# apple/ml-stable-diffusion

Hardware: NVIDIA H100
Metric: diffusion_iter_per_s (higher is better)
Workload: dtype f16

## Files before the change

### ml-stable-diffusion_b200/csrc/common.cuh

```cuda
#pragma once

#include <cuda.h>
#include <cuda_bf16.h>
#include <cuda_fp16.h>
#include <cuda_runtime.h>
#include <stdint.h>
#include <stdio.h>
#include <string.h>

namespace b200sd {

void set_error(const char* fmt, ...);

#define B200SD_CHECK_CUDA(expr)                                                            \
    do {                                                                                   \
        cudaError_t _e = (expr);                                                           \
        if (_e != cudaSuccess) {                                                           \
            ::b200sd::set_error("%s failed: %s (%s:%d)", #expr, cudaGetErrorString(_e),    \
                                __FILE__, __LINE__);                                       \
            return 1;                                                                      \
        }                                                                                  \
    } while (0)

#define B200SD_REQUIRE(cond, ...)                                                          \
    do {                                                                                   \
        if (!(cond)) {                                                                     \
            ::b200sd::set_error(__VA_ARGS__);                                              \
            return 2;                                                                      \
        }                                                                                  \
    } while (0)

int encode_tmap_f16(CUtensorMap* map, const void* base, int rank, const uint64_t* dims,
                    const uint64_t* strides_bytes, const uint32_t* box, const uint32_t* elem_strides);
int encode_tmap(CUtensorMap* map, CUtensorMapDataType dtype, const void* base, int rank, const uint64_t* dims,
                const uint64_t* strides_bytes, const uint32_t* box, const uint32_t* elem_strides,
                CUtensorMapSwizzle swizzle = CU_TENSOR_MAP_SWIZZLE_128B);

int num_sms();

bool pdl_enabled();

bool launch_class_enabled(int cls);

#ifdef __CUDACC__
template <typename... KArgs, typename... Args>
inline cudaError_t launch_kernel(void (*kernel)(KArgs...), dim3 grid, dim3 block, size_t smem, cudaStream_t stream,
                                 Args&&... args) {
    cudaLaunchConfig_t cfg;
    memset(&cfg, 0, sizeof(cfg));
    cfg.gridDim = grid;
    cfg.blockDim = block;
    cfg.dynamicSmemBytes = smem;
    cfg.stream = stream;
    cudaLaunchAttribute attr[1];
    if (pdl_enabled()) {
        attr[0].id = cudaLaunchAttributeProgrammaticStreamSerialization;
        attr[0].val.programmaticStreamSerializationAllowed = 1;
        cfg.attrs = attr;
        cfg.numAttrs = 1;
    }
    return cudaLaunchKernelEx(&cfg, kernel, static_cast<KArgs>(args)...);
}

__device__ __forceinline__ void pdl_wait() { asm volatile("griddepcontrol.wait;" ::: "memory"); }
__device__ __forceinline__ void pdl_trigger() { asm volatile("griddepcontrol.launch_dependents;" ::: "memory"); }

__device__ __forceinline__ uint32_t smem_u32(const void* p) {
    return static_cast<uint32_t>(__cvta_generic_to_shared(p));
}

__device__ __forceinline__ bool elect_one() {
    uint32_t pred = 0;
    asm volatile(
        "{\n\t"
        ".reg .pred P;\n\t"
        "elect.sync _|P, 0xffffffff;\n\t"
        "selp.u32 %0, 1, 0, P;\n\t"
        "}\n"
        : "=r"(pred));
    return pred != 0;
}

__device__ __forceinline__ void mbar_init(uint64_t* bar, uint32_t count) {
    asm volatile("mbarrier.init.shared::cta.b64 [%0], %1;" ::"r"(smem_u32(bar)), "r"(count));
}
__device__ __forceinline__ void fence_barrier_init() {
    asm volatile("fence.mbarrier_init.release.cluster;" ::: "memory");
}
__device__ __forceinline__ void fence_proxy_async_smem() {
    asm volatile("fence.proxy.async.shared::cta;" ::: "memory");
}
__device__ __forceinline__ void mbar_expect_tx(uint64_t* bar, uint32_t bytes) {
    asm volatile("mbarrier.arrive.expect_tx.shared::cta.b64 _, [%0], %1;" ::"r"(smem_u32(bar)), "r"(bytes)
                 : "memory");
}
__device__ __forceinline__ void mbar_arrive(uint64_t* bar) {
    asm volatile("mbarrier.arrive.shared::cta.b64 _, [%0];" ::"r"(smem_u32(bar)) : "memory");
}
__device__ __forceinline__ bool mbar_try_wait(uint64_t* bar, uint32_t parity) {
    uint32_t ok;
    asm volatile(
        "{\n\t"
        ".reg .pred P;\n\t"
        "mbarrier.try_wait.parity.shared::cta.b64 P, [%1], %2;\n\t"
        "selp.u32 %0, 1, 0, P;\n\t"
        "}\n"
        : "=r"(ok)
        : "r"(smem_u32(bar)), "r"(parity)
        : "memory");
    return ok != 0;
}
__device__ __forceinline__ void mbar_wait(uint64_t* bar, uint32_t parity) {
    while (!mbar_try_wait(bar, parity)) {
    }
}

__device__ __forceinline__ void prefetch_tmap(const CUtensorMap* m) {
    asm volatile("prefetch.tensormap [%0];" ::"l"(reinterpret_cast<uint64_t>(m)) : "memory");
}

static constexpr uint64_t kEvictNormal = 0x1000000000000000ull;
static constexpr uint64_t kEvictFirst = 0x12F0000000000000ull;
static constexpr uint64_t kEvictLast = 0x14F0000000000000ull;

__device__ __forceinline__ void tma_load_2d(void* smem_dst, const CUtensorMap* map, uint64_t* bar, int c0, int c1,
                                            uint64_t hint) {
    asm volatile(
        "cp.async.bulk.tensor.2d.shared::cluster.global.mbarrier::complete_tx::bytes.L2::cache_hint"
        " [%0], [%1, {%3, %4}], [%2], %5;" ::"r"(smem_u32(smem_dst)),
        "l"(reinterpret_cast<uint64_t>(map)), "r"(smem_u32(bar)), "r"(c0), "r"(c1), "l"(hint)
        : "memory");
}
__device__ __forceinline__ void tma_load_3d(void* smem_dst, const CUtensorMap* map, uint64_t* bar, int c0, int c1,
                                            int c2, uint64_t hint) {
    asm volatile(
        "cp.async.bulk.tensor.3d.shared::cluster.global.mbarrier::complete_tx::bytes.L2::cache_hint"
        " [%0], [%1, {%3, %4, %5}], [%2], %6;" ::"r"(smem_u32(smem_dst)),
        "l"(reinterpret_cast<uint64_t>(map)), "r"(smem_u32(bar)), "r"(c0), "r"(c1), "r"(c2), "l"(hint)
        : "memory");
}
__device__ __forceinline__ void tma_load_4d(void* smem_dst, const CUtensorMap* map, uint64_t* bar, int c0, int c1,
                                            int c2, int c3, uint64_t hint) {
    asm volatile(
        "cp.async.bulk.tensor.4d.shared::cluster.global.mbarrier::complete_tx::bytes.L2::cache_hint"
        " [%0], [%1, {%3, %4, %5, %6}], [%2], %7;" ::"r"(smem_u32(smem_dst)),
        "l"(reinterpret_cast<uint64_t>(map)), "r"(smem_u32(bar)), "r"(c0), "r"(c1), "r"(c2), "r"(c3), "l"(hint)
        : "memory");
}

__device__ __forceinline__ void wgmma_fence() { asm volatile("wgmma.fence.sync.aligned;" ::: "memory"); }
__device__ __forceinline__ void wgmma_commit() { asm volatile("wgmma.commit_group.sync.aligned;" ::: "memory"); }
template <int N>
__device__ __forceinline__ void wgmma_wait() {
    asm volatile("wgmma.wait_group.sync.aligned %0;" ::"n"(N) : "memory");
}
template <int N>
__device__ __forceinline__ void setmaxnreg_dec() {
    asm volatile("setmaxnreg.dec.sync.aligned.u32 %0;" ::"n"(N));
}
template <int N>
__device__ __forceinline__ void setmaxnreg_inc() {
    asm volatile("setmaxnreg.inc.sync.aligned.u32 %0;" ::"n"(N));
}
template <int R>
__device__ __forceinline__ void wgmma_fence_regs(float* d) {
#pragma unroll
    for (int i = 0; i < R; ++i) asm volatile("" : "+f"(d[i])::"memory");
}

#define B200SD_F8(i) "+f"(d[i]), "+f"(d[i + 1]), "+f"(d[i + 2]), "+f"(d[i + 3]), "+f"(d[i + 4]), "+f"(d[i + 5]), "+f"(d[i + 6]), "+f"(d[i + 7])
template <int N, typename T = __half>
__device__ __forceinline__ void wgmma_ss(float* d, uint64_t da, uint64_t db, uint32_t acc);
#define B200SD_WGMMA_SS(N, T, TY, REGS, IP, IA, IB, ...)                                                             \
    template <>                                                                                                      \
    __device__ __forceinline__ void wgmma_ss<N, T>(float* d, uint64_t da, uint64_t db, uint32_t acc) {               \
        asm volatile("{\n\t.reg .pred p;\n\tsetp.ne.b32 p, %" #IP ", 0;\n\t"                                          \
                     "wgmma.mma_async.sync.aligned.m64n" #N "k16.f32." TY "." TY " {" REGS "}, %" #IA ", %" #IB        \
                     ", p, 1, 1, 0, 0;\n\t}\n"                                                                         \
                     : __VA_ARGS__                                                                                   \
                     : "l"(da), "l"(db), "r"(acc)                                                                    \
                     : "memory");                                                                                    \
    }
#define B200SD_WGMMA_SS_BOTH(N, REGS, IP, IA, IB, ...)                  \
    B200SD_WGMMA_SS(N, __half, "f16", REGS, IP, IA, IB, __VA_ARGS__)   \
    B200SD_WGMMA_SS(N, __nv_bfloat16, "bf16", REGS, IP, IA, IB, __VA_ARGS__)
B200SD_WGMMA_SS_BOTH(16,
                     "%0, %1, %2, %3, %4, %5, %6, %7",
                     10, 8, 9, B200SD_F8(0))
B200SD_WGMMA_SS_BOTH(32,
                     "%0, %1, %2, %3, %4, %5, %6, %7, %8, %9, %10, %11, %12, %13, %14, %15",
                     18, 16, 17, B200SD_F8(0), B200SD_F8(8))
B200SD_WGMMA_SS_BOTH(64,
                     "%0, %1, %2, %3, %4, %5, %6, %7, %8, %9, %10, %11, %12, %13, %14, %15, "
                     "%16, %17, %18, %19, %20, %21, %22, %23, %24, %25, %26, %27, %28, %29, %30, %31",
                     34, 32, 33, B200SD_F8(0), B200SD_F8(8), B200SD_F8(16), B200SD_F8(24))
B200SD_WGMMA_SS_BOTH(96,
                     "%0, %1, %2, %3, %4, %5, %6, %7, %8, %9, %10, %11, %12, %13, %14, %15, "
                     "%16, %17, %18, %19, %20, %21, %22, %23, %24, %25, %26, %27, %28, %29, %30, %31, "
                     "%32, %33, %34, %35, %36, %37, %38, %39, %40, %41, %42, %43, %44, %45, %46, %47",
                     50, 48, 49, B200SD_F8(0), B200SD_F8(8), B200SD_F8(16), B200SD_F8(24), B200SD_F8(32), B200SD_F8(40))
B200SD_WGMMA_SS_BOTH(128,
                     "%0, %1, %2, %3, %4, %5, %6, %7, %8, %9, %10, %11, %12, %13, %14, %15, "
                     "%16, %17, %18, %19, %20, %21, %22, %23, %24, %25, %26, %27, %28, %29, %30, %31, "
                     "%32, %33, %34, %35, %36, %37, %38, %39, %40, %41, %42, %43, %44, %45, %46, %47, "
                     "%48, %49, %50, %51, %52, %53, %54, %55, %56, %57, %58, %59, %60, %61, %62, %63",
                     66, 64, 65, B200SD_F8(0), B200SD_F8(8), B200SD_F8(16), B200SD_F8(24), B200SD_F8(32), B200SD_F8(40), B200SD_F8(48), B200SD_F8(56))
B200SD_WGMMA_SS_BOTH(160,
                     "%0, %1, %2, %3, %4, %5, %6, %7, %8, %9, %10, %11, %12, %13, %14, %15, "
                     "%16, %17, %18, %19, %20, %21, %22, %23, %24, %25, %26, %27, %28, %29, %30, %31, "
                     "%32, %33, %34, %35, %36, %37, %38, %39, %40, %41, %42, %43, %44, %45, %46, %47, "
                     "%48, %49, %50, %51, %52, %53, %54, %55, %56, %57, %58, %59, %60, %61, %62, %63, "
                     "%64, %65, %66, %67, %68, %69, %70, %71, %72, %73, %74, %75, %76, %77, %78, %79",
                     82, 80, 81, B200SD_F8(0), B200SD_F8(8), B200SD_F8(16), B200SD_F8(24), B200SD_F8(32), B200SD_F8(40), B200SD_F8(48), B200SD_F8(56), B200SD_F8(64), B200SD_F8(72))
B200SD_WGMMA_SS_BOTH(192,
                     "%0, %1, %2, %3, %4, %5, %6, %7, %8, %9, %10, %11, %12, %13, %14, %15, "
                     "%16, %17, %18, %19, %20, %21, %22, %23, %24, %25, %26, %27, %28, %29, %30, %31, "
                     "%32, %33, %34, %35, %36, %37, %38, %39, %40, %41, %42, %43, %44, %45, %46, %47, "
                     "%48, %49, %50, %51, %52, %53, %54, %55, %56, %57, %58, %59, %60, %61, %62, %63, "
                     "%64, %65, %66, %67, %68, %69, %70, %71, %72, %73, %74, %75, %76, %77, %78, %79, "
                     "%80, %81, %82, %83, %84, %85, %86, %87, %88, %89, %90, %91, %92, %93, %94, %95",
                     98, 96, 97, B200SD_F8(0), B200SD_F8(8), B200SD_F8(16), B200SD_F8(24), B200SD_F8(32), B200SD_F8(40), B200SD_F8(48), B200SD_F8(56), B200SD_F8(64), B200SD_F8(72), B200SD_F8(80), B200SD_F8(88))
B200SD_WGMMA_SS_BOTH(256,
                     "%0, %1, %2, %3, %4, %5, %6, %7, %8, %9, %10, %11, %12, %13, %14, %15, "
                     "%16, %17, %18, %19, %20, %21, %22, %23, %24, %25, %26, %27, %28, %29, %30, %31, "
                     "%32, %33, %34, %35, %36, %37, %38, %39, %40, %41, %42, %43, %44, %45, %46, %47, "
                     "%48, %49, %50, %51, %52, %53, %54, %55, %56, %57, %58, %59, %60, %61, %62, %63, "
                     "%64, %65, %66, %67, %68, %69, %70, %71, %72, %73, %74, %75, %76, %77, %78, %79, "
                     "%80, %81, %82, %83, %84, %85, %86, %87, %88, %89, %90, %91, %92, %93, %94, %95, "
                     "%96, %97, %98, %99, %100, %101, %102, %103, %104, %105, %106, %107, %108, %109, %110, %111, "
                     "%112, %113, %114, %115, %116, %117, %118, %119, %120, %121, %122, %123, %124, %125, %126, %127",
                     130, 128, 129, B200SD_F8(0), B200SD_F8(8), B200SD_F8(16), B200SD_F8(24), B200SD_F8(32), B200SD_F8(40), B200SD_F8(48), B200SD_F8(56), B200SD_F8(64), B200SD_F8(72), B200SD_F8(80), B200SD_F8(88), B200SD_F8(96), B200SD_F8(104), B200SD_F8(112), B200SD_F8(120))
#undef B200SD_WGMMA_SS_BOTH
#undef B200SD_WGMMA_SS

template <int N>
__device__ __forceinline__ void wgmma_ss_s8(int32_t* d, uint64_t da, uint64_t db, uint32_t acc);
#define B200SD_I8(i) "+r"(d[i]), "+r"(d[i + 1]), "+r"(d[i + 2]), "+r"(d[i + 3]), "+r"(d[i + 4]), "+r"(d[i + 5]), "+r"(d[i + 6]), "+r"(d[i + 7])
#define B200SD_WGMMA_S8(N, REGS, IP, IA, IB, ...)                                                                    \
    template <>                                                                                                      \
    __device__ __forceinline__ void wgmma_ss_s8<N>(int32_t* d, uint64_t da, uint64_t db, uint32_t acc) {             \
        asm volatile("{\n\t.reg .pred p;\n\tsetp.ne.b32 p, %" #IP ", 0;\n\t"                                          \
                     "wgmma.mma_async.sync.aligned.m64n" #N "k32.s32.s8.s8 {" REGS "}, %" #IA ", %" #IB ", p;\n\t}\n"  \
                     : __VA_ARGS__                                                                                   \
                     : "l"(da), "l"(db), "r"(acc)                                                                    \
                     : "memory");                                                                                    \
    }
#define B200SD_R16 "%0, %1, %2, %3, %4, %5, %6, %7"
#define B200SD_R32 B200SD_R16 ", %8, %9, %10, %11, %12, %13, %14, %15"
#define B200SD_R64 B200SD_R32 ", %16, %17, %18, %19, %20, %21, %22, %23, %24, %25, %26, %27, %28, %29, %30, %31"
#define B200SD_R96 B200SD_R64 ", %32, %33, %34, %35, %36, %37, %38, %39, %40, %41, %42, %43, %44, %45, %46, %47"
#define B200SD_R128 B200SD_R96 ", %48, %49, %50, %51, %52, %53, %54, %55, %56, %57, %58, %59, %60, %61, %62, %63"
#define B200SD_R160 B200SD_R128 ", %64, %65, %66, %67, %68, %69, %70, %71, %72, %73, %74, %75, %76, %77, %78, %79"
#define B200SD_R192 B200SD_R160 ", %80, %81, %82, %83, %84, %85, %86, %87, %88, %89, %90, %91, %92, %93, %94, %95"
#define B200SD_R256 B200SD_R192 ", %96, %97, %98, %99, %100, %101, %102, %103, %104, %105, %106, %107, %108, %109, %110, " \
    "%111, %112, %113, %114, %115, %116, %117, %118, %119, %120, %121, %122, %123, %124, %125, %126, %127"
B200SD_WGMMA_S8(16, B200SD_R16, 10, 8, 9, B200SD_I8(0))
B200SD_WGMMA_S8(32, B200SD_R32, 18, 16, 17, B200SD_I8(0), B200SD_I8(8))
B200SD_WGMMA_S8(64, B200SD_R64, 34, 32, 33, B200SD_I8(0), B200SD_I8(8), B200SD_I8(16), B200SD_I8(24))
B200SD_WGMMA_S8(96, B200SD_R96, 50, 48, 49, B200SD_I8(0), B200SD_I8(8), B200SD_I8(16), B200SD_I8(24), B200SD_I8(32),
                B200SD_I8(40))
B200SD_WGMMA_S8(128, B200SD_R128, 66, 64, 65, B200SD_I8(0), B200SD_I8(8), B200SD_I8(16), B200SD_I8(24), B200SD_I8(32),
                B200SD_I8(40), B200SD_I8(48), B200SD_I8(56))
B200SD_WGMMA_S8(160, B200SD_R160, 82, 80, 81, B200SD_I8(0), B200SD_I8(8), B200SD_I8(16), B200SD_I8(24), B200SD_I8(32),
                B200SD_I8(40), B200SD_I8(48), B200SD_I8(56), B200SD_I8(64), B200SD_I8(72))
B200SD_WGMMA_S8(192, B200SD_R192, 98, 96, 97, B200SD_I8(0), B200SD_I8(8), B200SD_I8(16), B200SD_I8(24), B200SD_I8(32),
                B200SD_I8(40), B200SD_I8(48), B200SD_I8(56), B200SD_I8(64), B200SD_I8(72), B200SD_I8(80), B200SD_I8(88))
B200SD_WGMMA_S8(256, B200SD_R256, 130, 128, 129, B200SD_I8(0), B200SD_I8(8), B200SD_I8(16), B200SD_I8(24), B200SD_I8(32),
                B200SD_I8(40), B200SD_I8(48), B200SD_I8(56), B200SD_I8(64), B200SD_I8(72), B200SD_I8(80), B200SD_I8(88),
                B200SD_I8(96), B200SD_I8(104), B200SD_I8(112), B200SD_I8(120))
#undef B200SD_R256
#undef B200SD_R192
#undef B200SD_R160
#undef B200SD_R128
#undef B200SD_R96
#undef B200SD_R64
#undef B200SD_R32
#undef B200SD_R16
#undef B200SD_WGMMA_S8
#undef B200SD_I8
template <int R>
__device__ __forceinline__ void wgmma_fence_regs_s32(int32_t* d) {
#pragma unroll
    for (int i = 0; i < R; ++i) asm volatile("" : "+r"(d[i])::"memory");
}

__device__ __forceinline__ void wgmma_m64n64_rs_tb(float* d, const uint32_t (&a)[4], uint64_t db, uint32_t acc) {
    asm volatile(
        "{\n\t.reg .pred p;\n\tsetp.ne.b32 p, %37, 0;\n\t"
        "wgmma.mma_async.sync.aligned.m64n64k16.f32.f16.f16 "
        "{%0, %1, %2, %3, %4, %5, %6, %7, %8, %9, %10, %11, %12, %13, %14, %15, "
        "%16, %17, %18, %19, %20, %21, %22, %23, %24, %25, %26, %27, %28, %29, %30, %31}, "
        "{%32, %33, %34, %35}, %36, p, 1, 1, 1;\n\t}\n"
        : B200SD_F8(0), B200SD_F8(8), B200SD_F8(16), B200SD_F8(24)
        : "r"(a[0]), "r"(a[1]), "r"(a[2]), "r"(a[3]), "l"(db), "r"(acc)
        : "memory");
}
template <int N>
__device__ __forceinline__ void wgmma_rs_tb(float* d, const uint32_t (&a)[4], uint64_t db, uint32_t acc);
template <>
__device__ __forceinline__ void wgmma_rs_tb<64>(float* d, const uint32_t (&a)[4], uint64_t db, uint32_t acc) {
// ... 121 lines not shown
```

### ml-stable-diffusion_b200/csrc/norm.cu

```cuda
#include "common.cuh"
#include "../../include/b200sd.h"

#include <algorithm>
#include <cmath>
#include <cstdint>
#include <cooperative_groups.h>
#include <stdlib.h>

namespace b200sd {

extern void count_launch(int n);

static constexpr int kGnMaxImages = 1024;

template <typename T>
__device__ __forceinline__ void load8(const T* src, float (&f)[8]) {
    const uint4 raw = *reinterpret_cast<const uint4*>(src);
    const typename Elem16<T>::T2* h2 = reinterpret_cast<const typename Elem16<T>::T2*>(&raw);
#pragma unroll
    for (int q = 0; q < 4; ++q) {
        const float2 t = Elem16<T>::to_float2(h2[q]);
        f[2 * q] = t.x;
        f[2 * q + 1] = t.y;
    }
// ... 273 lines not shown
                                                const float* __restrict__ gamma, const float* __restrict__ beta, int silu,
                                                T* __restrict__ out, int8_t* __restrict__ out_s8, float inv_scale) {
    using E = Elem16<T>;
    namespace cg = cooperative_groups;
    cg::cluster_group cluster = cg::this_cluster();
    const int cs = gridDim.x, rank = blockIdx.x;
    const int C = c0 + c1, cpg = C / groups;
    const int vpr = chunk_ch >> 3;
    const int ng = chunk_ch / cpg;
    const int ch0 = blockIdx.y * chunk_ch;
    const int n = blockIdx.z;
    const int TY = blockDim.x / vpr;
    const int cv = threadIdx.x % vpr, ty = threadIdx.x / vpr;
    const bool active = ty < TY;
    const int px0 = rank * rows_per_cta, px1 = min(hw, px0 + rows_per_cta);
    const int ch = ch0 + cv * 8;
    const bool from0 = ch < c0;
    const int ld = from0 ? c0 : c1;
    const T* src = from0 ? x0 + static_cast<size_t>(n) * hw * c0 + ch : x1 + static_cast<size_t>(n) * hw * c1 + (ch - c0);

    extern __shared__ __align__(16) uint8_t csm[];
    uint4* slab = reinterpret_cast<uint4*>(csm);
    float* red = reinterpret_cast<float*>(slab + static_cast<size_t>(rows_per_cta) * vpr);
    float* chsum = red + 2 * TY * chunk_ch;
    float* xchg = chsum + 2 * chunk_ch;
    float* stat = xchg + 2 * ng;
    pdl_trigger();
    pdl_wait();

    float acc[8], acq[8];
#pragma unroll
    for (int e = 0; e < 8; ++e) acc[e] = acq[e] = 0.f;
    if (active) {
        for (int pxb = px0 + ty; pxb < px1; pxb += TY * kRowsInFlight) {
            uint4 raw[kRowsInFlight];
#pragma unroll
            for (int i = 0; i < kRowsInFlight; ++i) {
                const int px = pxb + i * TY;
                raw[i] = px < px1 ? __ldg(reinterpret_cast<const uint4*>(src + static_cast<size_t>(px) * ld)) : make_uint4(0, 0, 0, 0);
            }
#pragma unroll
            for (int i = 0; i < kRowsInFlight; ++i) {
                const int px = pxb + i * TY;
                if (px < px1) {
                    slab[(px - px0) * vpr + cv] = raw[i];
                    const typename E::T2* h2 = reinterpret_cast<const typename E::T2*>(&raw[i]);
#pragma unroll
                    for (int q = 0; q < 4; ++q) {
                        const float2 t = E::to_float2(h2[q]);
                        acc[2 * q] += t.x;
                        acc[2 * q + 1] += t.y;
                        acq[2 * q] = fmaf(t.x, t.x, acq[2 * q]);
                        acq[2 * q + 1] = fmaf(t.y, t.y, acq[2 * q + 1]);
                    }
                }
            }
        }
    }
    if (active) {
#pragma unroll
        for (int e = 0; e < 8; ++e) {
            red[(ty * 2) * chunk_ch + cv * 8 + e] = acc[e];
            red[(ty * 2 + 1) * chunk_ch + cv * 8 + e] = acq[e];
        }
    }
    __syncthreads();
    for (int i = threadIdx.x; i < 2 * chunk_ch; i += blockDim.x) {
        const int which = i / chunk_ch, c = i - which * chunk_ch;
        float a = 0.f;
        for (int r = 0; r < TY; ++r) a += red[(r * 2 + which) * chunk_ch + c];
        chsum[which * chunk_ch + c] = a;
    }
    __syncthreads();
    for (int i = threadIdx.x; i < 2 * ng; i += blockDim.x) {
        const int which = i / ng, g = i - which * ng;
        float a = 0.f;
        for (int c = 0; c < cpg; ++c) a += chsum[which * chunk_ch + g * cpg + c];
        xchg[which * ng + g] = a;
    }
    cluster.sync();
    const float inv_cnt = 1.0f / (static_cast<float>(hw) * static_cast<float>(cpg));
    for (int g = threadIdx.x; g < ng; g += blockDim.x) {
        float s = 0.f, q = 0.f;
        for (int r = 0; r < cs; ++r) {
            s += *cluster.map_shared_rank(&xchg[g], r);
            q += *cluster.map_shared_rank(&xchg[ng + g], r);
        }
        const float mean = s * inv_cnt;
        stat[g] = mean;
        stat[ng + g] = rsqrtf(fmaxf(q * inv_cnt - mean * mean, 0.f) + eps);
    }
    float mean8[8];
    cluster.barrier_arrive();
    __syncthreads();
#pragma unroll
    for (int e = 0; e < 8; ++e) mean8[e] = active ? stat[(cv * 8 + e) / cpg] : 0.f;
    if (active) {
        float sc8[8], sh8[8];
#pragma unroll
        for (int e = 0; e < 8; ++e) {
            const int g = (cv * 8 + e) / cpg;
            sc8[e] = stat[ng + g] * gamma[ch + e];
            sh8[e] = fmaf(-mean8[e], sc8[e], beta[ch + e]);
        }
        T* dst = kS8 ? nullptr : out + static_cast<size_t>(n) * hw * C + ch;
        int8_t* dst8 = kS8 ? out_s8 + static_cast<size_t>(n) * hw * C + ch : nullptr;
#pragma unroll 2
        for (int px = px0 + ty; px < px1; px += TY) {
            const uint4 raw = slab[(px - px0) * vpr + cv];
            const typename E::T2* h2 = reinterpret_cast<const typename E::T2*>(&raw);
            float f[8];
#pragma unroll
            for (int q = 0; q < 4; ++q) {
                const float2 t = E::to_float2(h2[q]);
                f[2 * q] = t.x;
                f[2 * q + 1] = t.y;
            }
#pragma unroll
            for (int e = 0; e < 8; ++e) {
                const float y = fmaf(f[e], sc8[e], sh8[e]);
                f[e] = silu ? __fdividef(y, 1.0f + __expf(-y)) : y;
            }
            if constexpr (kS8) {
                *reinterpret_cast<uint2*>(dst8 + static_cast<size_t>(px) * C) = quantize8_s8(f, inv_scale);
            } else {
                uint4 pk;
                pk.x = E::pack2(f[0], f[1]);
                pk.y = E::pack2(f[2], f[3]);
                pk.z = E::pack2(f[4], f[5]);
                pk.w = E::pack2(f[6], f[7]);
                *reinterpret_cast<uint4*>(dst + static_cast<size_t>(px) * C) = pk;
            }
        }
    }
    cluster.barrier_wait();
}

template <typename T, int kRowsInFlight>
__global__ void gn_cluster_kernel(const T* __restrict__ x0, const T* __restrict__ x1, int c0, int c1, int hw,
                                  int groups, int chunk_ch, int rows_per_cta, float eps,
                                  const float* __restrict__ gamma, const float* __restrict__ beta, int silu,
                                  T* __restrict__ out) {
    gn_cluster_body<T, kRowsInFlight, false>(x0, x1, c0, c1, hw, groups, chunk_ch, rows_per_cta, eps, gamma, beta, silu, out,
                                             nullptr, 0.f);
}

template <int kRowsInFlight>
__global__ void gn_cluster_s8_kernel(const __half* __restrict__ x0, const __half* __restrict__ x1, int c0, int c1, int hw,
                                     int groups, int chunk_ch, int rows_per_cta, float eps,
                                     const float* __restrict__ gamma, const float* __restrict__ beta, int silu,
                                     int8_t* __restrict__ out, float inv_scale) {
    gn_cluster_body<__half, kRowsInFlight, true>(x0, x1, c0, c1, hw, groups, chunk_ch, rows_per_cta, eps, gamma, beta, silu,
                                                 nullptr, out, inv_scale);
}

static int gn_chunks(int hw, int n_img) {
    (void)n_img;
    return std::max(1, std::min(128, hw / 16));
}

static unsigned int* gn_tickets() {
    static unsigned int* t = nullptr;
    if (!t) {
        if (cudaMalloc(&t, kGnMaxImages * sizeof(unsigned int)) != cudaSuccess) return nullptr;
        cudaMemset(t, 0, kGnMaxImages * sizeof(unsigned int));
    }
    return t;
}

template <int kVecsPerLane, bool kS8>
__device__ __forceinline__ void layer_norm_body(const __half* __restrict__ x, const float* __restrict__ gamma,
                                                const float* __restrict__ beta, __half* __restrict__ out,
                                                int8_t* __restrict__ out_s8, float inv_scale, int rows, int c, float eps) {
    const int warp = (blockIdx.x * blockDim.x + threadIdx.x) >> 5;
    const int lane = threadIdx.x & 31;
    if (warp >= rows) return;
    const int vecs = c / 8;
    const __half* src = x + static_cast<size_t>(warp) * c;
    float f[kVecsPerLane][8];
    float s = 0.f;
#pragma unroll
    for (int k = 0; k < kVecsPerLane; ++k) {
        const int v = lane + 32 * k;
        if (v < vecs) {
            const uint4 raw = *reinterpret_cast<const uint4*>(src + v * 8);
            const __half2* h2 = reinterpret_cast<const __half2*>(&raw);
#pragma unroll
            for (int q = 0; q < 4; ++q) {
                const float2 t = __half22float2(h2[q]);
                f[k][2 * q] = t.x;
                f[k][2 * q + 1] = t.y;
                s += t.x + t.y;
            }
        } else {
#pragma unroll
            for (int e = 0; e < 8; ++e) f[k][e] = 0.f;
        }
    }
#pragma unroll
    for (int o = 16; o > 0; o >>= 1) s += __shfl_xor_sync(0xffffffffu, s, o);
    const float mean = s / c;
    float sq = 0.f;
#pragma unroll
    for (int k = 0; k < kVecsPerLane; ++k) {
        const int v = lane + 32 * k;
        if (v < vecs) {
#pragma unroll
            for (int e = 0; e < 8; ++e) {
                const float d = f[k][e] - mean;
                sq += d * d;
            }
        }
    }
#pragma unroll
    for (int o = 16; o > 0; o >>= 1) sq += __shfl_xor_sync(0xffffffffu, sq, o);
    const float rstd = rsqrtf(sq / c + eps);
    __half* dst = kS8 ? nullptr : out + static_cast<size_t>(warp) * c;
#pragma unroll
    for (int k = 0; k < kVecsPerLane; ++k) {
        const int v = lane + 32 * k;
        if (v < vecs) {
            float y[8];
            const float4 g0 = *reinterpret_cast<const float4*>(gamma + v * 8);
            const float4 g1 = *reinterpret_cast<const float4*>(gamma + v * 8 + 4);
            const float4 b0 = *reinterpret_cast<const float4*>(beta + v * 8);
            const float4 b1 = *reinterpret_cast<const float4*>(beta + v * 8 + 4);
            const float gg[8] = {g0.x, g0.y, g0.z, g0.w, g1.x, g1.y, g1.z, g1.w};
            const float bb[8] = {b0.x, b0.y, b0.z, b0.w, b1.x, b1.y, b1.z, b1.w};
#pragma unroll
            for (int e = 0; e < 8; ++e) y[e] = (f[k][e] - mean) * rstd * gg[e] + bb[e];
            if constexpr (kS8) {
                *reinterpret_cast<uint2*>(out_s8 + static_cast<size_t>(warp) * c + v * 8) = quantize8_s8(y, inv_scale);
                continue;
            }
            uint4 pk;
            pk.x = pack_half2(y[0], y[1]);
            pk.y = pack_half2(y[2], y[3]);
            pk.z = pack_half2(y[4], y[5]);
            pk.w = pack_half2(y[6], y[7]);
            *reinterpret_cast<uint4*>(dst + v * 8) = pk;
        }
    }
}

template <int kVecsPerLane>
__global__ void __launch_bounds__(256) layer_norm_kernel(const __half* __restrict__ x, const float* __restrict__ gamma,
                                                         const float* __restrict__ beta, __half* __restrict__ out,
                                                         int rows, int c, float eps) {
    pdl_trigger();
    pdl_wait();
    layer_norm_body<kVecsPerLane, false>(x, gamma, beta, out, nullptr, 0.f, rows, c, eps);
}

template <int kVecsPerLane>
__global__ void __launch_bounds__(256) layer_norm_s8_kernel(const __half* __restrict__ x, const float* __restrict__ gamma,
                                                            const float* __restrict__ beta, int8_t* __restrict__ out,
                                                            float inv_scale, int rows, int c, float eps) {
    pdl_trigger();
    pdl_wait();
    layer_norm_body<kVecsPerLane, true>(x, gamma, beta, nullptr, out, inv_scale, rows, c, eps);
}


template <typename T>
__global__ void __launch_bounds__(256) softmax_rows_kernel(const float* __restrict__ in, T* __restrict__ out,
                                                           int cols, float scale_log2) {
    pdl_trigger();
    pdl_wait();
    const size_t row = blockIdx.x;
    const float* src = in + row * cols;
    T* dst = out + row * cols;
    __shared__ float red[8];
    float m = -INFINITY;
    for (int c = threadIdx.x; c < cols; c += blockDim.x) m = fmaxf(m, src[c] * scale_log2);
#pragma unroll
    for (int o = 16; o > 0; o >>= 1) m = fmaxf(m, __shfl_xor_sync(0xffffffffu, m, o));
    if ((threadIdx.x & 31) == 0) red[threadIdx.x >> 5] = m;
    __syncthreads();
    m = red[0];
    for (int i = 1; i < 8; ++i) m = fmaxf(m, red[i]);
    __syncthreads();
    float s = 0.f;
    for (int c = threadIdx.x; c < cols; c += blockDim.x) s += exp2f(src[c] * scale_log2 - m);
#pragma unroll
    for (int o = 16; o > 0; o >>= 1) s += __shfl_xor_sync(0xffffffffu, s, o);
    if ((threadIdx.x & 31) == 0) red[threadIdx.x >> 5] = s;
    __syncthreads();
    s = 0.f;
    for (int i = 0; i < 8; ++i) s += red[i];
    const float inv = 1.0f / s;
    for (int c = threadIdx.x; c < cols; c += blockDim.x) dst[c] = Elem16<T>::from_float(exp2f(src[c] * scale_log2 - m) * inv);
}

}

using namespace b200sd;

extern "C" size_t b200sd_group_norm_workspace_bytes(int32_t n_img, int32_t hw, int32_t c, int32_t groups) {
    (void)c;
    const size_t two_kernel = static_cast<size_t>(n_img) * gn_chunks(hw, n_img) * groups * 2 +
                              static_cast<size_t>(n_img) * groups * 2;
    return two_kernel * sizeof(float);
}

template <typename T>
static int group_norm(const void* x0, const void* x1, int32_t c0, int32_t c1, int32_t n_img, int32_t hw,
                      int32_t groups, float eps, const float* gamma, const float* beta, int32_t silu,
                      void* out, float* stats_ws, size_t stats_ws_bytes, void* stream_, int8_t* out_s8 = nullptr,
                      float inv_scale = 0.f) {
    if (!b200sd::launch_class_enabled(4)) return 0;
    cudaStream_t stream = static_cast<cudaStream_t>(stream_);
    const int C = c0 + c1;
    B200SD_REQUIRE(x0 && (out || out_s8) && gamma && beta && stats_ws, "b200sd_group_norm: null pointer");
    B200SD_REQUIRE(c0 > 0 && c0 % 8 == 0 && c1 >= 0 && c1 % 8 == 0 && (c1 == 0 || x1),
                   "b200sd_group_norm: channels must be multiples of 8 (c0=%d c1=%d)", c0, c1);
    B200SD_REQUIRE(groups > 0 && C % groups == 0, "b200sd_group_norm: %d channels not divisible by %d groups", C,
                   groups);
    B200SD_REQUIRE(n_img <= kGnMaxImages, "b200sd_group_norm: at most %d images per call", kGnMaxImages);
    B200SD_REQUIRE(stats_ws_bytes >= b200sd_group_norm_workspace_bytes(n_img, hw, C, groups),
                   "b200sd_group_norm: workspace too small");
    unsigned int* tickets = gn_tickets();
    B200SD_REQUIRE(tickets != nullptr, "b200sd_group_norm: could not allocate ticket counters");
    const int vecs = C / 8;
    B200SD_REQUIRE(vecs <= 384, "b200sd_group_norm: too many channels (%d)", C);
    {
        static int mode = -1;
        if (mode < 0) {
            const char* e = getenv("B200SD_GN_CLUSTER");
            mode = (e && e[0] == '0') ? 0 : 1;
        }
        const int cpg = C / groups;
        int chunk = cpg;
        while (chunk % 8 != 0) chunk += cpg;
        while (chunk < 32 && C % (2 * chunk) == 0) chunk *= 2;
        const int vpr = chunk / 8;
        const long clusters = static_cast<long>(C / chunk) * n_img;
        int cs = 8;
        while (cs > 1 && (hw / cs < 32 || clusters * cs > 4L * num_sms())) cs >>= 1;
        const int rows_per_cta = (hw + cs - 1) / cs;
        static int big_threads = -1;
        if (big_threads < 0) {
            const char* e = getenv("B200SD_GN_THREADS");
            big_threads = (e && atoi(e) == 512) ? 512 : 256;
        }
        const int threads = rows_per_cta >= 256 ? big_threads : 256;
        const int TY = threads / std::max(1, vpr);
        const size_t csmem = static_cast<size_t>(rows_per_cta) * vpr * 16 +
                             (2 * static_cast<size_t>(TY) * chunk + 2 * chunk + 4 * (chunk / cpg)) * sizeof(float);
        if (mode == 1 && vpr <= 64 && C % chunk == 0 && csmem <= 200 * 1024 && n_img <= 65535 && C / chunk <= 65535) {
            const int deep = (rows_per_cta + TY - 1) / TY >= 3 ? 1 : 0;
            auto kern = deep ? gn_cluster_kernel<T, 8> : gn_cluster_kernel<T, 2>;
            auto kern8 = deep ? gn_cluster_s8_kernel<8> : gn_cluster_s8_kernel<2>;
            static bool attr[2] = {false, false}, attr8[2] = {false, false};
            if (!(out_s8 ? attr8 : attr)[deep]) {
                if (out_s8) B200SD_CHECK_CUDA(cudaFuncSetAttribute(kern8, cudaFuncAttributeMaxDynamicSharedMemorySize, 200 * 1024));
                else B200SD_CHECK_CUDA(cudaFuncSetAttribute(kern, cudaFuncAttributeMaxDynamicSharedMemorySize, 200 * 1024));
                (out_s8 ? attr8 : attr)[deep] = true;
            }
            cudaLaunchConfig_t cfg;
            memset(&cfg, 0, sizeof(cfg));
            cfg.gridDim = dim3(cs, C / chunk, n_img);
            cfg.blockDim = dim3(threads);
            cfg.dynamicSmemBytes = csmem;
            cfg.stream = stream;
            cudaLaunchAttribute at[2];
            at[0].id = cudaLaunchAttributeClusterDimension;
            at[0].val.clusterDim.x = cs;
            at[0].val.clusterDim.y = 1;
            at[0].val.clusterDim.z = 1;
            cfg.attrs = at;
            cfg.numAttrs = 1;
            if (pdl_enabled()) {
                at[1].id = cudaLaunchAttributeProgrammaticStreamSerialization;
                at[1].val.programmaticStreamSerializationAllowed = 1;
                cfg.numAttrs = 2;
            }
            if (out_s8)
                B200SD_CHECK_CUDA(cudaLaunchKernelEx(&cfg, kern8, reinterpret_cast<const __half*>(x0),
                                                     reinterpret_cast<const __half*>(x1), static_cast<int>(c0),
                                                     static_cast<int>(c1), static_cast<int>(hw), static_cast<int>(groups), chunk,
                                                     rows_per_cta, eps, gamma, beta, static_cast<int>(silu), out_s8, inv_scale));
            else
                B200SD_CHECK_CUDA(cudaLaunchKernelEx(&cfg, kern, reinterpret_cast<const T*>(x0),
                                                     reinterpret_cast<const T*>(x1), static_cast<int>(c0),
                                                     static_cast<int>(c1), static_cast<int>(hw), static_cast<int>(groups), chunk,
                                                     rows_per_cta, eps, gamma, beta, static_cast<int>(silu),
                                                     reinterpret_cast<T*>(out)));
            B200SD_CHECK_CUDA(cudaGetLastError());
            count_launch(1);
            return 0;
        }
    }
    const int chunks = gn_chunks(hw, n_img);
    const int rows = std::max(1, std::min(256 / vecs, (hw + chunks - 1) / chunks));
    const int threads = (vecs * rows + 31) / 32 * 32;
    float* partial = stats_ws;
    float* final_stats = stats_ws + static_cast<size_t>(n_img) * chunks * groups * 2;
    const size_t smem1 = (static_cast<size_t>(rows) * C * 2 + static_cast<size_t>(C) * 2) * sizeof(float);
    static size_t smem1_static = SIZE_MAX, smem1_max = 0;
    if (smem1_static == SIZE_MAX) {
        cudaFuncAttributes fa;
        B200SD_CHECK_CUDA(cudaFuncGetAttributes(&fa, gn_stats_kernel<T>));
        smem1_static = fa.sharedSizeBytes;
    }
    if (smem1 + smem1_static > 48 * 1024 && smem1 > smem1_max) {
        B200SD_CHECK_CUDA(cudaFuncSetAttribute(gn_stats_kernel<T>, cudaFuncAttributeMaxDynamicSharedMemorySize,
                                               static_cast<int>(smem1)));
        smem1_max = smem1;
    }
    B200SD_CHECK_CUDA(launch_kernel(gn_stats_kernel<T>, dim3(dim3(chunks, n_img)), dim3(threads), smem1, stream, 
        reinterpret_cast<const T*>(x0), reinterpret_cast<const T*>(x1), c0, c1, hw, groups, chunks, rows, eps,
        partial, final_stats, tickets));
    B200SD_CHECK_CUDA(cudaGetLastError());
    const int want_blocks = std::max(1, (num_sms() * 4) / std::max(1, n_img));
    const int px_per_block = std::max(1, (hw + want_blocks - 1) / want_blocks);
    const int blocks = (hw + px_per_block - 1) / px_per_block;
    const size_t smem2 = 2 * static_cast<size_t>(C) * sizeof(float);
    if (out_s8)
        B200SD_CHECK_CUDA(launch_kernel(gn_apply_s8_kernel, dim3(dim3(blocks, n_img)), dim3(256), smem2, stream,
            reinterpret_cast<const __half*>(x0), reinterpret_cast<const __half*>(x1), c0, c1, hw, groups, final_stats,
            gamma, beta, silu, out_s8, inv_scale, px_per_block));
    else
        B200SD_CHECK_CUDA(launch_kernel(gn_apply_kernel<T>, dim3(dim3(blocks, n_img)), dim3(256), smem2, stream, 
            reinterpret_cast<const T*>(x0), reinterpret_cast<const T*>(x1), c0, c1, hw, groups, final_stats,
            gamma, beta, silu, reinterpret_cast<T*>(out), px_per_block));
    B200SD_CHECK_CUDA(cudaGetLastError());
    count_launch(2);
    return 0;
}

extern "C" int b200sd_group_norm(const void* x0, const void* x1, int32_t c0, int32_t c1, int32_t n_img, int32_t hw,
                                 int32_t groups, float eps, const float* gamma, const float* beta, int32_t silu,
                                 void* out, float* stats_ws, size_t stats_ws_bytes, void* stream) {
    return group_norm<__half>(x0, x1, c0, c1, n_img, hw, groups, eps, gamma, beta, silu, out, stats_ws, stats_ws_bytes, stream);
}

extern "C" int b200sd_group_norm_s8(const void* x0, const void* x1, int32_t c0, int32_t c1, int32_t n_img, int32_t hw,
                                    int32_t groups, float eps, const float* gamma, const float* beta, int32_t silu,
                                    float inv_scale, void* out, float* stats_ws, size_t stats_ws_bytes, void* stream) {
    B200SD_REQUIRE(out != nullptr, "b200sd_group_norm_s8: null pointer");
    B200SD_REQUIRE(std::isfinite(inv_scale) && inv_scale > 0.f, "b200sd_group_norm_s8: inv_scale=%g must be positive and finite",
                   static_cast<double>(inv_scale));
    return group_norm<__half>(x0, x1, c0, c1, n_img, hw, groups, eps, gamma, beta, silu, nullptr, stats_ws, stats_ws_bytes,
                              stream, static_cast<int8_t*>(out), inv_scale);
}

extern "C" int b200sd_group_norm_bf16(const void* x0, const void* x1, int32_t c0, int32_t c1, int32_t n_img, int32_t hw,
                                      int32_t groups, float eps, const float* gamma, const float* beta, int32_t silu,
                                      void* out, float* stats_ws, size_t stats_ws_bytes, void* stream) {
    return group_norm<__nv_bfloat16>(x0, x1, c0, c1, n_img, hw, groups, eps, gamma, beta, silu, out, stats_ws,
                                     stats_ws_bytes, stream);
}

extern "C" int b200sd_group_norm_apply(const void* x0, const void* x1, int32_t c0, int32_t c1, int32_t n_img, int32_t hw,
                                       int32_t groups, float eps, const float* chan0, const float* chan1,
                                       const float* gamma, const float* beta, int32_t silu, void* out, void* stream_) {
    if (!b200sd::launch_class_enabled(4)) return 0;
    cudaStream_t stream = static_cast<cudaStream_t>(stream_);
    const int C = c0 + c1;
    B200SD_REQUIRE(x0 && out && gamma && beta && chan0 && (c1 == 0 || (x1 && chan1)), "b200sd_group_norm_apply: null pointer");
    B200SD_REQUIRE(c0 > 0 && c0 % 8 == 0 && c1 >= 0 && c1 % 8 == 0 && groups > 0 && C % groups == 0 && n_img <= 65535,
                   "b200sd_group_norm_apply: bad channel / group counts (c0=%d c1=%d groups=%d)", c0, c1, groups);
    const int want_blocks = std::max(1, (num_sms() * 2) / std::max(1, n_img));
    const int px_per_block = std::max(1, (hw + want_blocks - 1) / want_blocks);
    const int blocks = (hw + px_per_block - 1) / px_per_block;
    const size_t smem = (2 * static_cast<size_t>(C) + 2 * groups) * sizeof(float);
    B200SD_REQUIRE(smem <= 48 * 1024, "b200sd_group_norm_apply: too many channels (%d)", C);
    B200SD_CHECK_CUDA(launch_kernel(gn_apply_chan_kernel, dim3(blocks, n_img), dim3(256), smem, stream,
                                    reinterpret_cast<const __half*>(x0), reinterpret_cast<const __half*>(x1), c0, c1, hw, groups, eps,
                                    chan0, chan1, gamma, beta, silu, reinterpret_cast<__half*>(out), px_per_block));
    B200SD_CHECK_CUDA(cudaGetLastError());
    count_launch(1);
    return 0;
}

extern "C" int b200sd_layer_norm(const void* x, const float* gamma, const float* beta, void* out, int32_t rows,
                                 int32_t c, float eps, void* stream_) {
    if (!b200sd::launch_class_enabled(4)) return 0;
    cudaStream_t stream = static_cast<cudaStream_t>(stream_);
    B200SD_REQUIRE(x && gamma && beta && out, "b200sd_layer_norm: null pointer");
    B200SD_REQUIRE(c % 8 == 0 && c > 0 && c <= 2048, "b200sd_layer_norm: c=%d must be a multiple of 8, <= 2048", c);
    const int vecs = c / 8;
    const int per_lane = (vecs + 31) / 32;
    const int blocks = (rows + 7) / 8;
    const __half* xi = reinterpret_cast<const __half*>(x);
    __half* xo = reinterpret_cast<__half*>(out);
    if (per_lane <= 2)
        B200SD_CHECK_CUDA(launch_kernel(layer_norm_kernel<2>, dim3(blocks), dim3(256), 0, stream, xi, gamma, beta, xo, rows, c, eps));
    else if (per_lane <= 5)
        B200SD_CHECK_CUDA(launch_kernel(layer_norm_kernel<5>, dim3(blocks), dim3(256), 0, stream, xi, gamma, beta, xo, rows, c, eps));
    else
        B200SD_CHECK_CUDA(launch_kernel(layer_norm_kernel<8>, dim3(blocks), dim3(256), 0, stream, xi, gamma, beta, xo, rows, c, eps));
    B200SD_CHECK_CUDA(cudaGetLastError());
    count_launch(1);
    return 0;
}

extern "C" int b200sd_layer_norm_s8(const void* x, const float* gamma, const float* beta, float inv_scale, void* out,
                                    int32_t rows, int32_t c, float eps, void* stream_) {
    if (!b200sd::launch_class_enabled(4)) return 0;
    cudaStream_t stream = static_cast<cudaStream_t>(stream_);
    B200SD_REQUIRE(x && gamma && beta && out, "b200sd_layer_norm_s8: null pointer");
// ... 37 lines not shown
```

Before: 162.1.

## Add TMA slab GroupNorm kernel for small spatial sizes

Adds a single-CTA GroupNorm path for hw<=256 that loads the whole channel-chunk slab into shared memory with one TMA tensor load, reduces the statistics, normalizes in place and writes the slab back with a TMA bulk store. This replaces the cluster-based kernel for small feature maps and avoids cluster launch and DSMEM reduction overhead. It covers the non-int8 case only and needs at least 32 clusters, and its large shared-memory use may limit occupancy.

```diff
diff --git a/ml-stable-diffusion_b200/csrc/common.cuh b/ml-stable-diffusion_b200/csrc/common.cuh
--- a/ml-stable-diffusion_b200/csrc/common.cuh
+++ b/ml-stable-diffusion_b200/csrc/common.cuh
@@ -146,6 +146,17 @@
         " [%0], [%1, {%3, %4, %5, %6}], [%2], %7;" ::"r"(smem_u32(smem_dst)),
         "l"(reinterpret_cast<uint64_t>(map)), "r"(smem_u32(bar)), "r"(c0), "r"(c1), "r"(c2), "r"(c3), "l"(hint)
         : "memory");
+}
+
+__device__ __forceinline__ void tma_store_3d(const CUtensorMap* map, const void* smem_src, int c0, int c1, int c2) {
+    asm volatile("cp.async.bulk.tensor.3d.global.shared::cta.bulk_group [%0, {%2, %3, %4}], [%1];" ::"l"(
+                     reinterpret_cast<uint64_t>(map)),
+                 "r"(smem_u32(smem_src)), "r"(c0), "r"(c1), "r"(c2)
+                 : "memory");
+}
+__device__ __forceinline__ void bulk_commit_group() { asm volatile("cp.async.bulk.commit_group;" ::: "memory"); }
+__device__ __forceinline__ void bulk_wait_group_read0() {
+    asm volatile("cp.async.bulk.wait_group.read 0;" ::: "memory");
 }
 
 __device__ __forceinline__ void wgmma_fence() { asm volatile("wgmma.fence.sync.aligned;" ::: "memory"); }
diff --git a/ml-stable-diffusion_b200/csrc/norm.cu b/ml-stable-diffusion_b200/csrc/norm.cu
--- a/ml-stable-diffusion_b200/csrc/norm.cu
+++ b/ml-stable-diffusion_b200/csrc/norm.cu
@@ -449,6 +449,170 @@
                                      int8_t* __restrict__ out, float inv_scale) {
     gn_cluster_body<__half, kRowsInFlight, true>(x0, x1, c0, c1, hw, groups, chunk_ch, rows_per_cta, eps, gamma, beta, silu,
                                                  nullptr, out, inv_scale);
+}
+
+static constexpr int kGnSlabThreads = 256;
+static constexpr int kGnSlabMaxRows = 256;
+
+struct GnSlabParams {
+    CUtensorMap tm_x0, tm_x1, tm_out;
+    const float* gamma;
+    const float* beta;
+    int c0, hw, cpg, chunk, silu;
+    float eps;
+};
+
+struct GnSlabSmem {
+    size_t red, red2, stat, bar, total;
+    __host__ __device__ GnSlabSmem(int esz, int hw, int chunk, int cpg) {
+        const int ty = kGnSlabThreads / (chunk / 8), runs = kGnSlabThreads / chunk > 1 ? kGnSlabThreads / chunk : 1;
+        red = (static_cast<size_t>(hw) * chunk * esz + 127) / 128 * 128;
+        red2 = red + 2 * static_cast<size_t>(ty) * chunk * sizeof(float);
+        stat = red2 + 2 * static_cast<size_t>(runs) * chunk * sizeof(float);
+        bar = (stat + 2 * static_cast<size_t>(chunk / cpg) * sizeof(float) + 7) / 8 * 8;
+        total = bar + sizeof(uint64_t);
+    }
+};
+
+template <typename T>
+__global__ void __launch_bounds__(kGnSlabThreads, 2) gn_slab_kernel(const __grid_constant__ GnSlabParams p) {
+    using E = Elem16<T>;
+    const int chunk = p.chunk, cpg = p.cpg, hw = p.hw;
+    const int vpr = chunk >> 3, ng = chunk / cpg;
+    const int ch0 = blockIdx.x * chunk, n = blockIdx.y;
+    const int TY = kGnSlabThreads / vpr;
+    const int tid = threadIdx.x, cv = tid % vpr, ty = tid / vpr;
+    const bool active = ty < TY;
+    const GnSlabSmem L(sizeof(T), hw, chunk, cpg);
+    extern __shared__ __align__(128) uint8_t ssm[];
+    T* slab = reinterpret_cast<T*>(ssm);
+    float* red = reinterpret_cast<float*>(ssm + L.red);
+    float* red2 = reinterpret_cast<float*>(ssm + L.red2);
+    float* stat = reinterpret_cast<float*>(ssm + L.stat);
+    uint64_t* bar = reinterpret_cast<uint64_t*>(ssm + L.bar);
+    const bool from0 = ch0 < p.c0;
+
+    if (tid == 0) {
+        prefetch_tmap(from0 ? &p.tm_x0 : &p.tm_x1);
+        prefetch_tmap(&p.tm_out);
+        mbar_init(bar, 1);
+        fence_barrier_init();
+    }
+    __syncthreads();
+    pdl_trigger();
+    pdl_wait();
+    if (tid == 0) {
+        mbar_expect_tx(bar, static_cast<uint32_t>(hw * chunk * sizeof(T)));
+        tma_load_3d(slab, from0 ? &p.tm_x0 : &p.tm_x1, bar, from0 ? ch0 : ch0 - p.c0, 0, n, kEvictNormal);
+    }
+    const int ch = ch0 + cv * 8;
+    float g8[8], b8[8];
+#pragma unroll
+    for (int e = 0; e < 8; ++e) {
+        g8[e] = active ? __ldg(p.gamma + ch + e) : 0.f;
+        b8[e] = active ? __ldg(p.beta + ch + e) : 0.f;
+    }
+    T* col = slab + cv * 8;
+
+    float acc[8], acq[8];
+#pragma unroll
+    for (int e = 0; e < 8; ++e) acc[e] = acq[e] = 0.f;
+    mbar_wait(bar, 0);
+    if (active) {
+#pragma unroll 4
+        for (int r = ty; r < hw; r += TY) {
+            const uint4 raw = *reinterpret_cast<const uint4*>(col + r * chunk);
+            const typename E::T2* h2 = reinterpret_cast<const typename E::T2*>(&raw);
+#pragma unroll
+            for (int q = 0; q < 4; ++q) {
+                const float2 t = E::to_float2(h2[q]);
+                acc[2 * q] += t.x;
+                acc[2 * q + 1] += t.y;
+                acq[2 * q] = fmaf(t.x, t.x, acq[2 * q]);
+                acq[2 * q + 1] = fmaf(t.y, t.y, acq[2 * q + 1]);
+            }
+        }
+#pragma unroll
+        for (int e = 0; e < 8; ++e) {
+            red[(ty * 2) * chunk + cv * 8 + e] = acc[e];
+            red[(ty * 2 + 1) * chunk + cv * 8 + e] = acq[e];
+        }
+    }
+    __syncthreads();
+    const int runs = kGnSlabThreads / chunk > 1 ? kGnSlabThreads / chunk : 1;
+    for (int i = tid; i < runs * chunk; i += kGnSlabThreads) {
+        const int s = i / chunk, c = i - s * chunk;
+        float a = 0.f, q = 0.f;
+        for (int t = s * TY / runs; t < (s + 1) * TY / runs; ++t) {
+            a += red[(t * 2) * chunk + c];
+            q += red[(t * 2 + 1) * chunk + c];
+        }
+        red2[(s * 2) * chunk + c] = a;
+        red2[(s * 2 + 1) * chunk + c] = q;
+    }
+    __syncthreads();
+    const int lane = tid & 31, warp = tid >> 5;
+    const float inv_cnt = 1.0f / (static_cast<float>(hw) * static_cast<float>(cpg));
+    for (int g = warp; g < ng; g += kGnSlabThreads / 32) {
+        float a = 0.f, q = 0.f;
+        for (int k = lane; k < runs * cpg; k += 32) {
+            const int s = k / cpg, c = g * cpg + (k - s * cpg);
+            a += red2[(s * 2) * chunk + c];
+            q += red2[(s * 2 + 1) * chunk + c];
+        }
+#pragma unroll
+        for (int off = 16; off > 0; off >>= 1) {
+            a += __shfl_xor_sync(0xffffffffu, a, off);
+            q += __shfl_xor_sync(0xffffffffu, q, off);
+        }
+        if (lane == 0) {
+            const float mean = a * inv_cnt;
+            stat[g] = mean;
+            stat[ng + g] = rsqrtf(fmaxf(q * inv_cnt - mean * mean, 0.f) + p.eps);
+        }
+    }
+    __syncthreads();
+
+    if (active) {
+        float sc8[8], sh8[8];
+#pragma unroll
+        for (int e = 0; e < 8; ++e) {
+            const int g = (cv * 8 + e) / cpg;
+            sc8[e] = stat[ng + g] * g8[e];
+            sh8[e] = fmaf(-stat[g], sc8[e], b8[e]);
+        }
+#pragma unroll 2
+        for (int r = ty; r < hw; r += TY) {
+            uint4* v = reinterpret_cast<uint4*>(col + r * chunk);
+            const uint4 raw = *v;
+            const typename E::T2* h2 = reinterpret_cast<const typename E::T2*>(&raw);
+            float f[8];
+#pragma unroll
+            for (int q = 0; q < 4; ++q) {
+                const float2 t = E::to_float2(h2[q]);
+                f[2 * q] = t.x;
+                f[2 * q + 1] = t.y;
+            }
+#pragma unroll
+            for (int e = 0; e < 8; ++e) {
+                const float y = fmaf(f[e], sc8[e], sh8[e]);
+                f[e] = p.silu ? __fdividef(y, 1.0f + __expf(-y)) : y;
+            }
+            uint4 pk;
+            pk.x = E::pack2(f[0], f[1]);
+            pk.y = E::pack2(f[2], f[3]);
+            pk.z = E::pack2(f[4], f[5]);
+            pk.w = E::pack2(f[6], f[7]);
+            *v = pk;
+        }
+    }
+    fence_proxy_async_smem();
+    __syncthreads();
+    if (tid == 0) {
+        tma_store_3d(&p.tm_out, slab, ch0, 0, n);
+        bulk_commit_group();
+        bulk_wait_group_read0();
+    }
 }
 
 static int gn_chunks(int hw, int n_img) {
@@ -645,6 +809,37 @@
         const size_t csmem = static_cast<size_t>(rows_per_cta) * vpr * 16 +
                              (2 * static_cast<size_t>(TY) * chunk + 2 * chunk + 4 * (chunk / cpg)) * sizeof(float);
         if (mode == 1 && vpr <= 64 && C % chunk == 0 && csmem <= 200 * 1024 && n_img <= 65535 && C / chunk <= 65535) {
+            if (!out_s8 && hw <= kGnSlabMaxRows && chunk <= kGnSlabMaxRows && (c1 == 0 || c0 % chunk == 0) &&
+                clusters >= 32) {
+                GnSlabParams p;
+                memset(&p, 0, sizeof(p));
+                const uint32_t box[3] = {static_cast<uint32_t>(chunk), static_cast<uint32_t>(hw), 1u};
+                const uint32_t one[3] = {1u, 1u, 1u};
+                auto map = [&](CUtensorMap* m, const void* base, int cols) {
+                    const uint64_t dims[3] = {static_cast<uint64_t>(cols), static_cast<uint64_t>(hw),
+                                              static_cast<uint64_t>(n_img)};
+                    const uint64_t strides[2] = {static_cast<uint64_t>(cols) * 2, static_cast<uint64_t>(hw) * cols * 2};
+                    return encode_tmap(m, CU_TENSOR_MAP_DATA_TYPE_FLOAT16, base, 3, dims, strides, box, one,
+                                       CU_TENSOR_MAP_SWIZZLE_NONE);
+                };
+                if (map(&p.tm_x0, x0, c0) != 0 || map(&p.tm_x1, c1 ? x1 : x0, c1 ? c1 : c0) != 0 ||
+                    map(&p.tm_out, out, C) != 0)
+                    return 2;
+                p.gamma = gamma, p.beta = beta, p.c0 = c0, p.hw = hw, p.cpg = cpg, p.chunk = chunk, p.silu = silu;
+                p.eps = eps;
+                const size_t smem = GnSlabSmem(sizeof(T), hw, chunk, cpg).total;
+                static bool slab_attr = false;
+                if (!slab_attr) {
+                    B200SD_CHECK_CUDA(cudaFuncSetAttribute(gn_slab_kernel<T>, cudaFuncAttributeMaxDynamicSharedMemorySize,
+                                                           200 * 1024));
+                    slab_attr = true;
+                }
+                B200SD_CHECK_CUDA(launch_kernel(gn_slab_kernel<T>, dim3(C / chunk, n_img), dim3(kGnSlabThreads), smem,
+                                                stream, p));
+                B200SD_CHECK_CUDA(cudaGetLastError());
+                count_launch(1);
+                return 0;
+            }
             const int deep = (rows_per_cta + TY - 1) / TY >= 3 ? 1 : 0;
             auto kern = deep ? gn_cluster_kernel<T, 8> : gn_cluster_kernel<T, 2>;
             auto kern8 = deep ? gn_cluster_s8_kernel<8> : gn_cluster_s8_kernel<2>;
```

New measurement: 163.8 (median of 6 runs). 1.0% higher.
